# wzjin2017/fhe-fed

Hardware: AMD Instinct MI355X
Metric: ciphertexts aggregated/sec (+ encode+enc / dec+decode ms), N clients, ring 2^15 L=4 (higher is better)
Workload: dtype u64; 1 GPU; cfg3: 16 learners/GPU x ResNet-18 (11689512 params -> 714 cts of 16384 slots), ring 2^15, L=4 towers; ring_dim=32768, towers=4, learners_total=16, cts_per_learner=714, parallelism=dp1 (one GPU, no collective), layout=arena

## Files before the change

fhe-fed_amd/csrc/kernels.hip:

```cpp
#include <hip/hip_runtime.h>

#include <algorithm>
#include <cmath>
#include <cstring>
#include <type_traits>
#include <vector>

#include "dev_common.h"
#include "shelfi_internal.h"

namespace shelfi {

static uint32_t xcd_combos(uint64_t G) {
  if (!switches().xcd_order) return 0;
  return (G % 8 == 0 && G <= 0xFFFFFFFFull) ? (uint32_t)G : 0;
}

template <int LOGR>
__global__ __launch_bounds__(256) void ntt_fwd_cols(uint64_t* __restrict__ polys, uint32_t L,
                                                    uint32_t logN, const uint64_t* __restrict__ tw,
                                                    const uint64_t* __restrict__ twp,
                                                    const TowerConst* __restrict__ tcs) {
  constexpr int R = 1 << LOGR;
  const uint32_t N = 1u << logN;
// ... 280 lines not shown
      const uint64_t e = (poly == 1 ? 0 : LN) + off + (last_g(r) << K4);
#pragma unroll
      for (int m = 0; m < ML; m += 2) {
        P[r][m / 2] = *reinterpret_cast<const ulonglong2*>(pk + e + m);
        Ps[r][m / 2] = *reinterpret_cast<const ulonglong2*>(pksh + e + m);
      }
    }
  };
  uint32_t k = blockIdx.x / ncombo;
  if (k < K) fetch(k, 0);
  __syncthreads();
  const auto lds_ld = [&](uint32_t, uint32_t pj) { return sm[pj]; };
  const auto mid_sync = [] {
    if (WL)
      wave_lds_sync();
    else
      __syncthreads();
  };
#pragma unroll 1
  for (; k < K; k += per_combo) {
#pragma unroll 1
    for (int poly = 0; poly < 3; ++poly) {
      uint64_t x[NS1][M1];
      if (VT && poly == 0) {
#pragma unroll
        for (int m = 0; m < M1; ++m) {
          const uint32_t w = (uint32_t)pf[0][m];
          x[0][m] = vts[w & 127u] + vts[81 + ((w >> 7) & 127u)] + vts[162 + ((w >> 14) & 127u)] + vts[243 + (w >> 21)];
        }
      } else {
#pragma unroll
        for (int r = 0; r < NS1; ++r)
#pragma unroll
          for (int m = 0; m < M1; ++m) x[r][m] = pf[r][m];
      }
      if (poly < 2)
        fetch(k, poly + 1);
      else if (k + per_combo < K)
        fetch(k + per_combo, 0);
      if (poly > 0) fetch_key(poly);
#pragma unroll
      for (int r = 0; r < NS1; ++r)
        fwd_set_ct<BL, BL - 1, K1, NR>(x[r], 0u, tws, q, n8q);
      if (WL) __syncthreads();
#pragma unroll
      for (int r = 0; r < NS1; ++r) {
        const uint32_t p0 = lpad(threadIdx.x + 256u * r);
#pragma unroll
        for (int m = 0; m < M1; ++m) sm[p0 + lofs<(1 << D1)>(m)] = x[r][m];
      }
      __syncthreads();
      fwd_chunk_ct<BL, BL - 1 - K1, K2, NR>(tws, q, n8q, lds_ld, [&](int, uint32_t, uint32_t pj0, auto& y) {
#pragma unroll
        for (int m = 0; m < (1 << K2); ++m) sm[pj0 + lofs<(1 << (BL - K1 - K2))>(m)] = y[m];
      });
      mid_sync();
      fwd_chunk_ct<BL, BL - 1 - K1 - K2, K3, NR>(tws, q, n8q, lds_ld, [&](int, uint32_t, uint32_t pj0, auto& y) {
#pragma unroll
        for (int m = 0; m < (1 << K3); ++m) sm[pj0 + lofs<(1 << (BL - K1 - K2 - K3))>(m)] = y[m];
      });
      mid_sync();
#pragma unroll
      for (int r = 0; r < NSL; ++r) {
        const uint32_t g = last_g(r), j0 = g << K4, pj0 = lpad(j0);
        uint64_t y[ML];
#pragma unroll
        for (int m = 0; m < ML; ++m) y[m] = sm[pj0 + m];
        fwd_set_ct<BL, K4 - 1, K4, NR>(y, g, tws, q, n8q);
        if (poly == 0) {
#pragma unroll
          for (int m = 0; m < ML; ++m) V[r][m] = y[m];
        } else {
          uint64_t* __restrict__ dst = ct + ((uint64_t)k * 2 + (poly - 1)) * LN + off + j0;
#pragma unroll
          for (int m = 0; m < ML; m += 2) {
            ulonglong2 c;
            c.x = red_any(shoup_lazy(V[r][m], P[r][m / 2].x, Ps[r][m / 2].x, q) + y[m], cst);
            c.y = red_any(shoup_lazy(V[r][m + 1], P[r][m / 2].y, Ps[r][m / 2].y, q) + y[m + 1], cst);
            *reinterpret_cast<ulonglong2*>(dst + m) = c;
          }
        }
      }
      if (!WL) __syncthreads();
    }
  }
}

template <int BL, int K1, int K2, int K3, int K4, bool SUM = false>
__global__ __launch_bounds__(256) void ntt_inv_blocks_dec_ct(uint64_t* __restrict__ dbuf, uint32_t L,
                                                             uint32_t logN,
                                                             const ulonglong2* __restrict__ twb,
                                                             const TowerConst* __restrict__ tcs,
                                                             const uint64_t* __restrict__ ct,
                                                             const uint64_t* __restrict__ sk,
                                                             const uint64_t* __restrict__ sksh,
                                                             uint32_t xg, uint32_t ctL) {
  static_assert(K1 + K2 + K3 + K4 == BL, "chunk plan must cover the block");
  __shared__ __attribute__((aligned(16))) uint64_t sm[lpad_size(BL)];
  const uint32_t sstart = logN - BL;
  const uint32_t bid = xcd_block(blockIdx.x, xg);
  const uint32_t b = bid & ((1u << sstart) - 1);
  const uint32_t poly = bid >> sstart;
  const uint32_t t = poly % L, k = poly / L;
  const TowerConst& cst = tcs[t];
  const uint64_t q = cst.q, n4q = cst.n4q, n8q = cst.n8q;
  const ulonglong2* __restrict__ tb = twb + ((uint64_t)t << logN) + ((uint64_t)b << BL);
  const uint64_t off = ((uint64_t)t << logN) + ((uint64_t)b << BL);
  const uint64_t LN = (uint64_t)L << logN;
  const uint64_t CLN = (uint64_t)ctL << logN;
  const uint64_t* __restrict__ c0 = ct + (uint64_t)k * 2 * CLN + off;
  const uint64_t* __restrict__ c1 = c0 + CLN;
  const uint64_t* __restrict__ s = sk + off;
  const uint64_t* __restrict__ ss = sksh + off;
  const auto lds_ld = [&](uint32_t, uint32_t pj) { return sm[pj]; };
  inv_chunk_ct<BL, 0, K1, false>(tb, q, n8q,
                          [&](uint32_t j, uint32_t) {
                            const uint64_t a0 = SUM ? red_any(c0[j], cst) : c0[j];
                            return csub_neg(a0 + shoup_lazy(c1[j], s[j], ss[j], q), n4q);
                          },
                          [&](int, uint32_t, uint32_t pj0, auto& x) {
#pragma unroll
                            for (int m = 0; m < (1 << K1); ++m) sm[pj0 + lofs<1>(m)] = x[m];
                          });
  __syncthreads();
  inv_chunk_ct<BL, K1, K2, true>(tb, q, n8q, lds_ld, [&](int, uint32_t, uint32_t pj0, auto& x) {
#pragma unroll
    for (int m = 0; m < (1 << K2); ++m) sm[pj0 + lofs<(1 << K1)>(m)] = x[m];
  });
  __syncthreads();
  inv_chunk_ct<BL, K1 + K2, K3, true>(tb, q, n8q, lds_ld, [&](int, uint32_t, uint32_t pj0, auto& x) {
#pragma unroll
    for (int m = 0; m < (1 << K3); ++m) sm[pj0 + lofs<(1 << (K1 + K2))>(m)] = x[m];
  });
  __syncthreads();
  uint64_t* __restrict__ dst = dbuf + (uint64_t)k * LN + off;
  inv_chunk_ct<BL, BL - K4, K4, true>(tb, q, n8q, lds_ld, [&](int, uint32_t j0, uint32_t, auto& x) {
#pragma unroll
    for (int m = 0; m < (1 << K4); ++m) dst[j0 + (m << (BL - K4))] = x[m];
  });
}

template <int BL, int K1, int K2, int K3, int K4, bool SUM = false, bool WL = false>
__global__ __launch_bounds__(256) void ntt_inv_blocks_dec_pp(uint64_t* __restrict__ dbuf, uint32_t L,
                                                             uint32_t logN,
                                                             const ulonglong2* __restrict__ twb,
                                                             const TowerConst* __restrict__ tcs,
                                                             const uint64_t* __restrict__ ct,
                                                             const uint64_t* __restrict__ sk,
                                                             const uint64_t* __restrict__ sksh, uint32_t K,
                                                             uint32_t per_combo, uint32_t ctL) {
  static_assert(K1 + K2 + K3 + K4 == BL, "chunk plan must cover the block");
  constexpr int M1 = 1 << K1, NS1 = (1 << (BL - K1)) / 256;
  static_assert(!WL || (BL == 11 && K1 == 2 && K2 == 3 && K3 == 3 && K4 == 3), "wave-local plan");
  __shared__ __attribute__((aligned(16))) ulonglong2 tws[1 << BL];
  __shared__ __attribute__((aligned(16))) uint64_t sm[lpad_size(BL)];
  const auto first_g = [&](int r) -> uint32_t {
    return WL ? ((threadIdx.x >> 6) * (64u * NS1) + 64u * r + (threadIdx.x & 63u)) : threadIdx.x + 256u * r;
  };
  const uint32_t sstart = logN - BL;
  const uint32_t ncombo = L << sstart;
  const uint32_t combo = blockIdx.x % ncombo;
  const uint32_t b = combo & ((1u << sstart) - 1), t = combo >> sstart;
  const TowerConst& cst = tcs[t];
  const uint64_t q = cst.q, n4q = cst.n4q, n8q = cst.n8q;
  const uint64_t off = ((uint64_t)t << logN) + ((uint64_t)b << BL);
  const uint64_t LN = (uint64_t)L << logN;
// ... 396 lines not shown
      smc[i0 + lenh] = cmul(csub(a0, a1), W);
    }
    __syncthreads();
  }
  for (uint32_t i = threadIdx.x; i < blk; i += 256) buf[off + i] = smc[i];
}

template <int KC, int A>
__device__ __forceinline__ void fft_dit_set(double2 (&v)[1 << KC], uint32_t l, const double2* __restrict__ tw) {
#pragma unroll
  for (int i = 0; i < KC; ++i) {
#pragma unroll
    for (int m0 = 0; m0 < (1 << KC); ++m0) {
      if (m0 & (1 << i)) continue;
      const int m1 = m0 + (1 << i);
      const double2 W = tw[(1u << (A + i)) + l + ((uint32_t)(m0 & ((1 << i) - 1)) << A)];
      const double2 u = v[m0];
      const double2 w = cmul(v[m1], W);
      v[m0] = cadd(u, w);
      v[m1] = csub(u, w);
    }
  }
}
template <int KC, int A>
__device__ __forceinline__ void fft_dif_set(double2 (&v)[1 << KC], uint32_t l, const double2* __restrict__ tw) {
#pragma unroll
  for (int i = KC - 1; i >= 0; --i) {
#pragma unroll
    for (int m0 = 0; m0 < (1 << KC); ++m0) {
      if (m0 & (1 << i)) continue;
      const int m1 = m0 + (1 << i);
      const double2 W = tw[(1u << (A + i)) + l + ((uint32_t)(m0 & ((1 << i) - 1)) << A)];
      const double2 a0 = v[m0], a1 = v[m1];
      v[m0] = cadd(a0, a1);
      v[m1] = cmul(csub(a0, a1), W);
    }
  }
}
template <int BL, int KC, int A, bool DIT, class Load, class Store>
__device__ __forceinline__ void fft_chunk(const double2* __restrict__ tw, Load ld, Store st) {
  constexpr int T = 1 << (BL - 3), NS = (1 << (BL - KC)) / T;
  static_assert(NS >= 1, "chunk plan");
#pragma unroll
  for (int r = 0; r < NS; ++r) {
    const uint32_t s = threadIdx.x + (uint32_t)T * r;
    const uint32_t l = s & ((1u << A) - 1), j0 = ((s >> A) << (A + KC)) | l;
    double2 v[1 << KC];
#pragma unroll
    for (int m = 0; m < (1 << KC); ++m) v[m] = ld(j0 + ((uint32_t)m << A));
    if (DIT)
      fft_dit_set<KC, A>(v, l, tw);
    else
      fft_dif_set<KC, A>(v, l, tw);
#pragma unroll
    for (int m = 0; m < (1 << KC); ++m) st(j0 + ((uint32_t)m << A), v[m]);
  }
}
template <bool SWZ = true>
__device__ __forceinline__ uint32_t fft_swz(uint32_t j) { return SWZ ? j ^ ((j >> 3) & 15u) : j; }

template <int BL, int K1, int K2, int K3, int K4, bool SWZ = true>
__global__ __launch_bounds__(1 << (BL - 3)) void fft_inv_blocks_ct(double2* __restrict__ buf, uint32_t logS,
                                                                  const double2* __restrict__ tw) {
  static_assert(K1 + K2 + K3 + K4 == BL, "chunk plan");
  __shared__ __attribute__((aligned(16))) double2 sm[1 << BL];
  const uint32_t S = 1u << logS, sh = logS - BL;
  const uint64_t k = blockIdx.x >> sh;
  const uint32_t b = blockIdx.x & ((1u << sh) - 1);
  double2* __restrict__ g = buf + k * S + ((uint64_t)b << BL);
  const auto lds_ld = [&](uint32_t j) { return sm[fft_swz<SWZ>(j)]; };
  const auto lds_st = [&](uint32_t j, double2 v) { sm[fft_swz<SWZ>(j)] = v; };
  fft_chunk<BL, K1, BL - K1, false>(tw, [&](uint32_t j) { return g[j]; }, lds_st);
  __syncthreads();
  fft_chunk<BL, K2, BL - K1 - K2, false>(tw, lds_ld, lds_st);
  __syncthreads();
  fft_chunk<BL, K3, BL - K1 - K2 - K3, false>(tw, lds_ld, lds_st);
  __syncthreads();
  fft_chunk<BL, K4, 0, false>(tw, lds_ld, [&](uint32_t j, double2 v) { g[j] = v; });
}

constexpr uint32_t kFftWholeLogS = 14;
constexpr uint64_t kFftWholeMinK = 128;
constexpr uint64_t kEncNoredMinK = 192;
constexpr uint64_t kDecPpMinItems = 4096;
constexpr uint32_t kFftWholeRow = 1088;
__device__ __forceinline__ uint32_t fft_wpad(uint32_t e) { return e + (e >> 5); }
__device__ __forceinline__ uint32_t fft_wt1(uint32_t l, int m) { return 4 * l + (l >> 3) + 264u * (m >> 2) + (m & 3); }
__device__ __forceinline__ uint32_t fft_wx3(uint32_t l, int m) { return l + (l >> 5) + 66u * m; }
__device__ __forceinline__ uint32_t fft_xa1(uint32_t l, int m) { return 4 * l + (l >> 2) + 272u * (m >> 2) + (m & 3); }
__device__ __forceinline__ uint32_t fft_xa2(uint32_t l, int m) { return 68 * (l >> 2) + (l & 3) + 4u * m + (m >> 2); }
__device__ __forceinline__ uint32_t fft_xb2(uint32_t l, int m) {
  return 68 * (l >> 2) + (l & 3) + 4u * m + 2u * (m >> 3);
}
__device__ __forceinline__ uint32_t fft_xb3(uint32_t l, int m) { return l + 2 * (l >> 5) + 68u * m; }

template <class PF, class QF>
__device__ __forceinline__ void fft_wave_xch(double2 (&a)[16], double* __restrict__ Ls, PF P, QF Q) {
#pragma unroll
  for (int m = 0; m < 16; ++m) Ls[P(m)] = a[m].x;
  wave_lds_sync();
#pragma unroll
  for (int m = 0; m < 16; ++m) a[m].x = Ls[Q(m)];
  wave_lds_sync();
#pragma unroll
  for (int m = 0; m < 16; ++m) Ls[P(m)] = a[m].y;
  wave_lds_sync();
#pragma unroll
  for (int m = 0; m < 16; ++m) a[m].y = Ls[Q(m)];
  wave_lds_sync();
}

template <bool TO_BLOCKS>
__device__ __forceinline__ void fft_whole_transpose(double2 (&a)[16], double* __restrict__ lds) {
  const uint32_t T = threadIdx.x, w = T >> 6, l = T & 63;
#pragma unroll
  for (int part = 0; part < 2; ++part) {
#pragma unroll
    for (int i = 0; i < 16; ++i) {
      const double v = part ? a[i].y : a[i].x;
      if (TO_BLOCKS)
        lds[i * kFftWholeRow + fft_wpad(T)] = v;
      else
        lds[w * kFftWholeRow + fft_wx3(l, i)] = v;
    }
    __syncthreads();
#pragma unroll
    for (int i = 0; i < 16; ++i) {
      const double v = TO_BLOCKS ? lds[w * kFftWholeRow + fft_wx3(l, i)] : lds[i * kFftWholeRow + fft_wpad(T)];
      if (part)
        a[i].y = v;
      else
        a[i].x = v;
    }
    __syncthreads();
  }
}

__global__ __launch_bounds__(1024) void fft_inv_whole(const double* __restrict__ x, uint64_t n,
                                                      double2* __restrict__ buf, const double2* __restrict__ tw) {
  constexpr uint32_t S = 1u << kFftWholeLogS, BLK = 1024;
  constexpr int R = 16;
  __shared__ double lds[16 * kFftWholeRow];
  const uint64_t k = blockIdx.x;
  const uint32_t T = threadIdx.x, w = T >> 6, l = T & 63;
  double2 a[R];
  const double* __restrict__ xk = x + k * S;
  const uint32_t rem = n > k * S ? (uint32_t)std::min<uint64_t>(n - k * S, S) : 0u;
#pragma unroll
  for (int r = 0; r < R; ++r) {
    const uint32_t i = T + (uint32_t)r * BLK;
    a[r] = make_double2(i < rem ? xk[i] : 0.0, 0.0);
  }
#pragma unroll
  for (int s = 0; s < 4; ++s) {
    asm volatile("" ::: "memory");
    const uint32_t lenh = (S >> s) >> 1;
    const int trr = R >> (s + 1);
#pragma unroll
    for (int r0 = 0; r0 < R; ++r0) {
      if ((r0 / trr) % 2) continue;
      const int r1 = r0 + trr;
      const double2 W = tw[lenh + T + (uint32_t)(r0 & ((R >> s) - 1)) * BLK];
      const double2 u = cadd(a[r0], a[r1]);
      const double2 d = csub(a[r0], a[r1]);
      a[r0] = u;
      a[r1] = cmul(d, W);
// ... 461 lines not shown
void launch_encrypt(const Params& p, const DeviceTables& dt, const DeviceKeys& dk, const double* x,
                    uint64_t n, uint64_t K, uint64_t* ct, void* scratch, const uint32_t key[8],
                    uint64_t g0, GenFlag flag, hipStream_t s) {
  if (!K) return;
  const uint32_t logS = __builtin_ctz(p.batch);
  double2* fbuf = reinterpret_cast<double2*>(scratch);
  uint64_t* pbuf = reinterpret_cast<uint64_t*>(fbuf + K * (uint64_t)p.batch);
  launch_encode_fft(p, dt, x, n, K, fbuf, s);
  Key8 k8;
  for (int i = 0; i < 8; ++i) k8.k[i] = key[i];
  const Switches& sw = switches();
  const uint32_t nblkLog = ntt_block_log(p.logN);
  const int nlogR = (int)(p.logN - nblkLog);
  const bool fused = (nlogR == 3 || nlogR == 4 || (nlogR == 5 && sw.enc_tab && sw.enc_x5)) && dt.enc_tab &&
                     sw.enc_fused;
  int64_t* me0 = reinterpret_cast<int64_t*>(pbuf + K * 3ull * p.L * p.N);
  int16_t* ve = reinterpret_cast<int16_t*>(me0 + K * (uint64_t)p.N);
  const bool pp = fused && nblkLog == 11 && dt.red_ok && sw.enc_pp;
  uint32_t t_split = 0;
  while (t_split < p.L && p.q[t_split] >= kNoRedQ) ++t_split;
  for (uint32_t t = t_split; t < p.L; ++t)
    if (p.q[t] >= kNoRedQ) t_split = p.L;
  if (!pp || !sw.enc_nored || K < kEncNoredMinK || nlogR == 5) t_split = p.L;
  bool vt = false;
  if (fused) {
    const uint64_t nb = (K << (p.logN - (nlogR == 5 ? 4 : nlogR))) / 256;
    const bool tab = sw.enc_tab;
#define ENC_COLS(LR, TB, ...)                                                                                   \
  hipLaunchKernelGGL((enc_cols_fused<LR, TB, ##__VA_ARGS__>), dim3((uint32_t)nb), dim3(256), 0, s, fbuf, K, p.logN, logS, p.L, \
                     p.delta, dt.cdt, dt.cdt_len, k8, g0, dt.tc, dt.psi_rev, dt.psi_rev_sh, pbuf, flag, t_split,  \
                     dt.enc_tab)
    const bool ts = nlogR == 4 && tab && p.L == 4 && (sw.enc_ts >= 0 ? sw.enc_ts == 1 : K <= kEncTsMaxK);
    vt = pp && tab && !ts && nlogR == 4 && dt.enc_vtab && sw.enc_vt && ntt_wave_local();
    if (nlogR == 5)
      ENC_COLS(4, true, 3, true, false, false, true);
    else if (vt)
      ENC_COLS(4, true, 3, true, false, true);
    else if (ts)
      hipLaunchKernelGGL((enc_cols_fused<4, true, 3, true, true>), dim3((uint32_t)(nb * 4)), dim3(256), 0, s, fbuf, K,
                         p.logN, logS, p.L, p.delta, dt.cdt, dt.cdt_len, k8, g0, dt.tc, dt.psi_rev, dt.psi_rev_sh,
                         pbuf, flag, t_split, dt.enc_tab);
    else if (nlogR == 3 && tab)
      ENC_COLS(3, true);
    else if (nlogR == 3)
      ENC_COLS(3, false);
    else if (tab)
      ENC_COLS(4, true, 3, true);
    else
      ENC_COLS(4, false);
#undef ENC_COLS
    SHELFI_HIP(hipGetLastError());
  } else {
    const uint64_t threads = K * (p.N / 16);
    hipLaunchKernelGGL(enc_prep_kernel, dim3((uint32_t)((threads + 255) / 256)), dim3(256), 0, s, fbuf,
                       K, p.logN, logS, p.delta, dt.cdt, dt.cdt_len, k8, g0, me0, ve, flag);
    SHELFI_HIP(hipGetLastError());
  }
  if (nlogR > 0 && !fused) {
    const uint64_t nb = K * ((p.N >> nlogR) / 256);
#define COLS_ENC(LR)                                                                          \
  hipLaunchKernelGGL((ntt_fwd_cols_enc<LR, 0>), dim3((uint32_t)nb), dim3(256), 0, s, me0, ve, K,  \
                     p.logN, p.L, dt.tc, dt.psi_rev, dt.psi_rev_sh, pbuf);                       \
  hipLaunchKernelGGL((ntt_fwd_cols_enc<LR, 1>), dim3((uint32_t)nb), dim3(256), 0, s, me0, ve, K,  \
                     p.logN, p.L, dt.tc, dt.psi_rev, dt.psi_rev_sh, pbuf);                       \
  hipLaunchKernelGGL((ntt_fwd_cols_enc<LR, 2>), dim3((uint32_t)nb), dim3(256), 0, s, me0, ve, K,  \
                     p.logN, p.L, dt.tc, dt.psi_rev, dt.psi_rev_sh, pbuf);
    switch (nlogR) {
      case 1: COLS_ENC(1) break;
      case 2: COLS_ENC(2) break;
      case 3: COLS_ENC(3) break;
      case 4: COLS_ENC(4) break;
      case 5: COLS_ENC(5) break;
      case 6: COLS_ENC(6) break;
      default: throw Error{SHELFI_ERR_ARG, "unsupported ring dimension"};
    }
#undef COLS_ENC
    SHELFI_HIP(hipGetLastError());
  }
  const uint64_t nbb = K * p.L << nlogR;
  if (nbb > 0x7FFFFFFFull) throw Error{SHELFI_ERR_ARG, "encrypt batch too large"};
  const uint32_t xg = xcd_combos(p.L << nlogR);
  if (pp) {
    const bool wl = ntt_wave_local();
    const auto launch_pp = [&](uint32_t ta, uint32_t nt, bool nr) {
      const uint32_t ncombo = nt << nlogR;
      const uint32_t pc = pp_per_combo(ncombo, K, 3);
#define ENC_PP(NR, WL, VT)                                                                                       \
  hipLaunchKernelGGL((ntt_fwd_blocks_enc_pp<11, 3, 3, 3, 2, NR, WL, VT>), dim3(ncombo * pc), dim3(256), 0, s, pbuf, \
                     p.L, p.logN, dt.tw_fwd_blk, dt.tc, dk.pk, dk.pk_sh, ct, (uint32_t)K, pc, ta, nt, dt.enc_vtab)
      if (nr && wl && vt) ENC_PP(true, true, true);
      else if (nr && wl) ENC_PP(true, true, false);
      else if (nr) ENC_PP(true, false, false);
      else if (wl && vt) ENC_PP(false, true, true);
      else if (wl) ENC_PP(false, true, false);
      else ENC_PP(false, false, false);
#undef ENC_PP
    };
    if (t_split > 0) launch_pp(0u, t_split, false);
    if (t_split < p.L) launch_pp(t_split, p.L - t_split, true);
  } else if (nlogR > 0 && nblkLog == 11 && dt.red_ok)
    hipLaunchKernelGGL((ntt_fwd_blocks_enc_ct<11, 3, 3, 3, 2>), dim3((uint32_t)nbb), dim3(256), 0, s,
                       pbuf, p.L, p.logN, dt.tw_fwd_blk, dt.tc, dk.pk, dk.pk_sh, ct, 0u, xg);
  else if (nlogR > 0 && nblkLog == 12 && dt.red_ok)
    hipLaunchKernelGGL((ntt_fwd_blocks_enc_ct<12, 3, 3, 3, 3>), dim3((uint32_t)nbb), dim3(256), 0, s,
                       pbuf, p.L, p.logN, dt.tw_fwd_blk, dt.tc, dk.pk, dk.pk_sh, ct, 0u, xg);
  else if (nblkLog > 11)
    hipLaunchKernelGGL(ntt_fwd_blocks_enc<8>, dim3((uint32_t)nbb), dim3(256), sizeof(uint64_t) << nblkLog, s,
                     pbuf, p.L, p.logN, (uint32_t)nlogR, dt.psi_rev, dt.psi_rev_sh, dt.tc, dk.pk,
                     dk.pk_sh, ct, nlogR > 0 ? (const int64_t*)nullptr : me0,
                     nlogR > 0 ? (const int16_t*)nullptr : ve);
  else
    hipLaunchKernelGGL(ntt_fwd_blocks_enc<4>, dim3((uint32_t)nbb), dim3(256), sizeof(uint64_t) << nblkLog, s,
                     pbuf, p.L, p.logN, (uint32_t)nlogR, dt.psi_rev, dt.psi_rev_sh, dt.tc, dk.pk,
                     dk.pk_sh, ct, nlogR > 0 ? (const int64_t*)nullptr : me0,
                     nlogR > 0 ? (const int16_t*)nullptr : ve);
  SHELFI_HIP(hipGetLastError());
}

__device__ __forceinline__ int64_t enc_fit_wrap(int64_t r) {
  constexpr int64_t kMax64 = 9223372036854775295LL;
  constexpr int64_t hf = kMax64 >> 1;
  if (r > hf) return r - kMax64;
  if (r < 0 && kMax64 + r <= hf) return r + kMax64;
  return r;
}

__global__ __launch_bounds__(256) void enc_maxabs_kernel(const double2* __restrict__ fbuf, uint32_t logS,
                                                         uint64_t* __restrict__ amax) {
  const uint32_t S = 1u << logS;
  const double2* __restrict__ f = fbuf + (uint64_t)blockIdx.x * S;
  uint64_t m = 0;
  for (uint32_t i = threadIdx.x; i < S; i += 256) {
    const double2 v = f[i];
    const uint64_t a = (uint64_t)__double_as_longlong(fabs(v.x)), b = (uint64_t)__double_as_longlong(fabs(v.y));
    m = max(m, max(a, b));
  }
  __shared__ uint64_t red[256];
  red[threadIdx.x] = m;
  __syncthreads();
  for (uint32_t w = 128; w; w >>= 1) {
    if (threadIdx.x < w) red[threadIdx.x] = max(red[threadIdx.x], red[threadIdx.x + w]);
    __syncthreads();
  }
  if (threadIdx.x == 0) amax[blockIdx.x] = red[0];
}

__global__ __launch_bounds__(256) void enc_expand_approx_kernel(
    const double2* __restrict__ fbuf, uint64_t K, uint32_t logN, uint32_t logS, uint32_t L, double delta,
    const uint64_t* __restrict__ cdt, int T, Key8 key, uint64_t g0, const TowerConst* __restrict__ tcs,
    const int32_t* __restrict__ log_approx, const uint64_t* __restrict__ pw, uint64_t* __restrict__ pbuf) {
  const uint32_t N = 1u << logN, S = 1u << logS, N16 = N >> 4, V0 = N >> 6;
  __shared__ uint32_t thi[64], tlo[64];
  load_cdt32(cdt, T, thi, tlo);
  __syncthreads();
  const uint64_t gid = (uint64_t)blockIdx.x * 256 + threadIdx.x;
  const uint64_t k = gid >> (logN - 4);
  if (k >= K) return;
  const uint32_t h = (uint32_t)(gid & (N16 - 1));
  const uint64_t nonce = (1ull << 56) | (g0 + k);
  const uint32_t half = N >> 1, gapLog = logN - 1 - logS;
  const double dS = (double)S;
  const double approx = ldexp(1.0, log_approx[k]);
  uint32_t w[16];
  chacha20_block32(key, h >> 2, nonce, w);
  uint32_t u[4] = {w[4 * (h & 3)], w[4 * (h & 3) + 1], w[4 * (h & 3) + 2], w[4 * (h & 3) + 3]};
  int32_t vv[16], e0[16], e1[16];
  int64_t mm[16];
#pragma unroll
// ... 1099 lines not shown
```

fhe-fed_amd/csrc/shelfi_internal.h:

```cpp
#pragma once

#include <hip/hip_runtime.h>

#include <cstdint>
#include <cstdlib>
#include <mutex>
#include <string>
#include <vector>

#include "../../include/shelfi.h"

namespace shelfi {

typedef unsigned __int128 u128;

void set_error(const std::string& msg);
struct Error {
  int code;
  std::string msg;
};
#define SHELFI_HIP(expr)                                                             \
  do {                                                                               \
    hipError_t _e = (expr);                                                          \
    if (_e != hipSuccess)                                                            \
      throw ::shelfi::Error{SHELFI_ERR_DEVICE, std::string(#expr) + ": " +           \
                                                 hipGetErrorString(_e)};             \
  } while (0)

constexpr int kMaxTowers = 16;
constexpr int kMaxCommRanks = 16;
constexpr int kFftBlockLog = 10;
constexpr int kFftBlockLogBig = 11;
inline uint32_t fft_block_log(uint32_t logS) {
  const uint32_t b = logS >= 15 ? (uint32_t)kFftBlockLogBig : (uint32_t)kFftBlockLog;
  return logS < b ? logS : b;
}
constexpr int kNttBlockLog = 11;
constexpr int kNttBlockLogBig = 12;
inline uint32_t ntt_block_log(uint32_t logN) {
  static const uint32_t ovr = [] {
    const char* e = std::getenv("SHELFI_NTT_BLOCK_LOG_BIG");
    const int v = e ? std::atoi(e) : 0;
    return (uint32_t)((v == 11 || v == 12) ? v : 0);
  }();
  uint32_t b = logN >= 17 ? (uint32_t)kNttBlockLogBig : (uint32_t)kNttBlockLog;
  if (ovr && logN >= 16) b = ovr;
  return logN < b ? logN : b;
}

struct Switches {
  bool xcd_order = true;
  bool ntt_wl = true;
  bool fft_ct = true;
  bool fft_whole = true;
  bool enc_fused = true;
  bool enc_pp = true;
  bool dec_pp = true;
  bool enc_nored = true;
  bool enc_tab = true;
  bool enc_vt = true;
  int enc_ts = -1;
  bool dec_all_towers = false;
  bool stage_trace = false;
  bool enc_x5 = true;
  int pack_kernel = 0;
  int pack_unroll = 0;
  int pack_waves = 0;
  int wavg_rows = 0;
  uint32_t wavg_strands = 0;
  int arena_stager = -1;
  uint64_t dev_chunk_mib = 4096;
  uint64_t wavg_chunk_mib = 0;
  uint64_t stage_slot_mib = 16;
  bool h2d_direct = false;
  bool h2d_two = true;
};
const Switches& switches();
void reload_switches();

struct Params {
  uint32_t N = 0, logN = 0, L = 0, batch = 0, gap = 0, scale_bits = 0, first_mod_bits = 0;
  uint64_t q[kMaxTowers] = {0};
  uint64_t psi[kMaxTowers] = {0};
  double delta = 0.0;
  double sigma = 3.19;
};

uint64_t powmod(uint64_t a, uint64_t e, uint64_t q);
uint64_t invmod(uint64_t a, uint64_t q);
uint64_t shoup(uint64_t w, uint64_t q);
uint64_t mod_signed(int64_t v, uint64_t q);
bool is_prime(uint64_t n);
uint32_t default_ring_dim(uint32_t L, uint32_t scale_bits, uint32_t first_mod_bits, uint32_t batch);
uint32_t hybrid_dnum(uint32_t L);
double ring_dim_qbound(uint32_t L, uint32_t scale_bits, uint32_t first_mod_bits);
void generate_chain(uint32_t N, uint32_t L, uint32_t scale_bits, uint32_t first_mod_bits,
                    uint64_t* q, uint64_t* psi);
uint64_t min_root(uint64_t m, uint64_t q);
void special_primes(uint32_t N, uint32_t L, const uint64_t* q, uint32_t* dnum, uint32_t* alpha,
                    uint32_t* kP, uint64_t* p, uint64_t* ppsi);
void fft_twiddles(uint32_t slots, double* inv_re, double* inv_im, double* fwd_re, double* fwd_im);
int gauss_cdt(double sigma, uint64_t* cdt, int max_entries);
uint64_t fnv1a(const void* data, size_t n, uint64_t h = 1469598103934665603ull);

struct TowerConst {
  uint64_t q;
  uint64_t one_shoup;
  uint64_t r30, r30_shoup;
  uint64_t r60, r60_shoup;
  uint64_t r64, r64_shoup;
  uint64_t ninv, ninv_shoup;
  uint64_t qhat_inv, qhat_inv_shoup;
  double inv_q;
  uint64_t nq, n4q, n8q;
  uint32_t red_r, red_sh, red_ok;
  uint32_t crt_sh;
  float inv_q32;
  uint32_t pad32;
  uint64_t bq62;
  uint64_t ninv_qhat, ninv_qhat_shoup;
  uint64_t ninv_qhat_w1, ninv_qhat_w1_shoup;
  uint32_t crt30[7], nq30[7];
  uint64_t crt_edge[2];
};

constexpr int kEncVTab = 4 * 81, kEncETab = 128, kEncTab = kEncVTab + kEncETab;

struct DeviceTables {
  TowerConst* tc = nullptr;
  uint64_t* psi_rev = nullptr;
  uint64_t* psi_rev_sh = nullptr;
  uint64_t* ipsi_rev = nullptr;
  uint64_t* ipsi_rev_sh = nullptr;
  ulonglong2* tw_fwd_blk = nullptr;
  ulonglong2* tw_inv_blk = nullptr;
  bool red_ok = false;
  double2* fft_inv = nullptr;
  double2* fft_fwd = nullptr;
  uint64_t* cdt = nullptr;
// ... 226 lines not shown
```

fhe-fed_amd/csrc/switches.cpp:

```cpp
#include <atomic>
#include <cstdlib>
#include <cstring>
#include <initializer_list>

#include "shelfi_internal.h"

namespace shelfi {

static std::atomic<const Switches*> g_switches{nullptr};

static bool env_flag(const char* name, char off_or_on, bool dflt) {
  const char* e = getenv(name);
  return e && *e == off_or_on ? !dflt : dflt;
}
static int env_choice(const char* name, std::initializer_list<int> allowed, int dflt) {
  const char* e = getenv(name);
  if (!e) return dflt;
  const int v = atoi(e);
  for (int a : allowed)
    if (a == v) return v;
  return dflt;
}

void reload_switches() {
  Switches s;
  s.xcd_order = env_flag("SHELFI_XCD_ORDER", '0', true);
  s.ntt_wl = env_flag("SHELFI_NTT_WL", '0', true);
  s.fft_ct = env_flag("SHELFI_FFT_CT", '0', true);
  s.fft_whole = env_flag("SHELFI_FFT_WHOLE", '0', true);
  s.enc_fused = env_flag("SHELFI_ENC_FUSED_COLS", '0', true);
  s.enc_pp = env_flag("SHELFI_ENC_PP", '0', true);
  s.dec_pp = env_flag("SHELFI_DEC_PP", '0', true);
  s.enc_nored = env_flag("SHELFI_ENC_NORED", '0', true);
  s.enc_tab = env_flag("SHELFI_ENC_TAB", '0', true);
  s.enc_vt = env_flag("SHELFI_ENC_VT", '0', true);
  s.enc_ts = env_choice("SHELFI_ENC_TS", {0, 1}, -1);
  s.dec_all_towers = env_flag("SHELFI_DEC_ALL_TOWERS", '1', false);
  s.enc_x5 = env_flag("SHELFI_ENC_X5", '0', true);
  s.stage_trace = env_choice("SHELFI_STAGE_TRACE", {0, 1}, 0) == 1;
  if (const char* e = getenv("SHELFI_PACK_KERNEL")) s.pack_kernel = !strcmp(e, "v4") ? 4 : !strcmp(e, "r3") ? 3 : 0;
  s.pack_unroll = env_choice("SHELFI_PACK_UNROLL", {1, 2, 4, 8}, 0);
  s.pack_waves = env_choice("SHELFI_PACK_WAVES", {2, 8}, 0);
  s.wavg_rows = env_choice("SHELFI_WAVG_ROWS", {1, 2}, 0);
  if (const char* e = getenv("SHELFI_WAVG_STRANDS"))
    if (atoi(e) > 1 && atoi(e) <= 4096) s.wavg_strands = (uint32_t)atoi(e);
  s.arena_stager = env_choice("SHELFI_ARENA_STAGER", {0, 1}, -1);
  if (const char* e = getenv("SHELFI_DEV_CHUNK_MIB"))
    if (atoll(e) > 0) s.dev_chunk_mib = (uint64_t)atoll(e);
  if (const char* e = getenv("SHELFI_WAVG_CHUNK_MIB"))
    if (atoll(e) > 0) s.wavg_chunk_mib = (uint64_t)atoll(e);
  if (const char* e = getenv("SHELFI_STAGE_SLOT_MIB"))
    if (atoll(e) > 0 && atoll(e) <= 256) s.stage_slot_mib = (uint64_t)atoll(e);
  s.h2d_direct = env_flag("SHELFI_H2D_DIRECT", '1', false);
  s.h2d_two = env_flag("SHELFI_H2D_TWO", '0', true);
  g_switches.store(new Switches(s), std::memory_order_release);
}
const Switches& switches() { return *g_switches.load(std::memory_order_acquire); }
static const bool g_switches_read = (reload_switches(), true);

}

extern "C" {

void shelfi_reload_switches(void) { shelfi::reload_switches(); }

}
```

Baseline: 3.355 million client-ciphertexts/s.

## Add two-ciphertext-per-block encrypt NTT kernel sharing staged twiddles in LDS

Adds a 512-thread variant of the persistent encrypt forward-NTT kernel in which two 256-thread halves each process a different ciphertext. Both halves share one LDS copy of the block twiddles and value table, and the first-stage twiddles now come from LDS rather than global memory. The variant is picked by default when ring logR equals 4 and the batch holds at least 32 ciphertexts, and an env switch can override it. The goal is to halve per-ciphertext twiddle staging and global twiddle traffic and to improve occupancy through a fixed waves-per-EU hint, at the cost of more LDS per block and extra block-wide syncs.

```diff
diff --git a/fhe-fed_amd/csrc/kernels.hip b/fhe-fed_amd/csrc/kernels.hip
--- a/fhe-fed_amd/csrc/kernels.hip
+++ b/fhe-fed_amd/csrc/kernels.hip
@@ -386,6 +386,162 @@
         }
       }
       if (!WL) __syncthreads();
+    }
+  }
+}
+
+template <int BL, int K1, int K2, int K3, int K4, bool NR, bool VT>
+__global__ __launch_bounds__(512) __attribute__((amdgpu_waves_per_eu(4, 4))) void ntt_fwd_blocks_enc_pp2(
+    const uint64_t* __restrict__ pbuf, uint32_t L, uint32_t logN, const ulonglong2* __restrict__ twb,
+    const TowerConst* __restrict__ tcs, const uint64_t* __restrict__ pk, const uint64_t* __restrict__ pksh,
+    uint64_t* __restrict__ ct, uint32_t K, uint32_t per_combo, uint32_t t0, uint32_t nt,
+    const uint64_t* __restrict__ vtab) {
+  static_assert(BL == 11 && K1 == 3 && K2 == 3 && K3 == 3 && K4 == 2, "wave-local plan");
+  constexpr int M1 = 1 << K1, D1 = BL - K1;
+  constexpr int ML = 1 << K4, NSL = (1 << (BL - K4)) / 256;
+  struct Lds {
+    uint64_t vts[VT ? 4 * 81 : 2];
+    ulonglong2 tws[1 << BL];
+    uint64_t sm2[2 * lpad_size(BL)];
+  };
+  static_assert(sizeof(uint64_t[VT ? 4 * 81 : 2]) % 16 == 0, "tws stays 16-byte aligned");
+  __shared__ __attribute__((aligned(16))) Lds lds;
+  uint64_t* const vts = lds.vts;
+  ulonglong2* const tws = lds.tws;
+  uint64_t* const sm2 = lds.sm2;
+  const uint32_t h = __builtin_amdgcn_readfirstlane(threadIdx.x >> 8), tid = threadIdx.x & 255u;
+  const auto otid = [&]() -> uint32_t {
+    uint32_t tl = tid;
+    asm volatile("" : "+v"(tl));
+    return tl & 255u;
+  };
+  constexpr int DL2 = BL - K1 - K2, DL3 = BL - K1 - K2 - K3;
+  const uint32_t hb = h * lpad_size(BL);
+  const uint32_t pj1 = hb + lpad(tid);
+  const uint32_t pj2 = hb + lpad(((tid >> DL2) << (DL2 + K2)) + (tid & ((1u << DL2) - 1)));
+  const uint32_t pj3 = hb + lpad(((tid >> DL3) << (DL3 + K3)) + (tid & ((1u << DL3) - 1)));
+  const uint32_t pjl = hb + lpad(((tid >> 6) * (64u * NSL) + (tid & 63u)) << K4);
+  constexpr uint32_t kLastStep = (64u << K4) + ((64u << K4) >> 3);
+  const auto last_g = [](uint32_t tl, int r) -> uint32_t { return (tl >> 6) * (64u * NSL) + 64u * r + (tl & 63u); };
+  const uint32_t sstart = logN - BL;
+  const uint32_t ncombo = nt << sstart;
+  const uint32_t combo = blockIdx.x % ncombo;
+  const uint32_t b = combo & ((1u << sstart) - 1), t = t0 + (combo >> sstart);
+  const TowerConst& cst = tcs[t];
+  const uint64_t q = cst.q, n8q = cst.n8q;
+  const uint64_t off = ((uint64_t)t << logN) + ((uint64_t)b << BL);
+  const uint64_t LN = (uint64_t)L << logN;
+  {
+    const ulonglong2* __restrict__ src = twb + off;
+    for (uint32_t i = threadIdx.x; i < (1u << BL); i += 512) tws[i] = src[i];
+    if (VT)
+      for (uint32_t i = threadIdx.x; i < 4 * 81; i += 512) vts[i] = vtab[((uint64_t)t * 16 + b) * (4 * 81) + i];
+  }
+  uint64_t pf[M1];
+  uint64_t V[NSL][ML];
+  const auto fetch = [&](uint32_t kk, int poly) {
+    const uint32_t tl = otid();
+    if (VT && poly == 0) {
+      const uint32_t* __restrict__ vp = reinterpret_cast<const uint32_t*>(pbuf + (uint64_t)kk * 3 * LN);
+#pragma unroll
+      for (int m = 0; m < M1; ++m) pf[m] = (vp + (m << D1))[tl];
+      return;
+    }
+    const uint64_t* __restrict__ src = pbuf + ((uint64_t)kk * 3 + poly) * LN + off;
+#pragma unroll
+    for (int m = 0; m < M1; ++m) pf[m] = __builtin_nontemporal_load((src + (m << D1)) + tl);
+  };
+  const uint32_t stride = 2 * per_combo;
+  uint32_t k0 = 2 * (blockIdx.x / ncombo);
+  if (k0 + h < K) fetch(k0 + h, 0);
+  __syncthreads();
+#pragma unroll 1
+  for (; k0 < K; k0 += stride) {
+    const uint32_t k = k0 + h;
+    const bool act = k < K;
+#pragma unroll 1
+    for (int poly = 0; poly < 3; ++poly) {
+      uint64_t x[M1];
+      if (act) {
+        if (VT && poly == 0) {
+#pragma unroll
+          for (int m = 0; m < M1; ++m) {
+            const uint32_t w = (uint32_t)pf[m];
+            x[m] = vts[w & 127u] + vts[81 + ((w >> 7) & 127u)] + vts[162 + ((w >> 14) & 127u)] + vts[243 + (w >> 21)];
+          }
+        } else {
+#pragma unroll
+          for (int m = 0; m < M1; ++m) x[m] = pf[m];
+        }
+        if (poly < 2)
+          fetch(k, poly + 1);
+        else if (k + stride < K)
+          fetch(k + stride, 0);
+        fwd_set_ct<BL, BL - 1, K1, NR>(x, 0u, tws, q, n8q);
+      }
+      __syncthreads();
+      if (act) {
+#pragma unroll
+        for (int m = 0; m < M1; ++m) sm2[pj1 + lofs<(1 << D1)>(m)] = x[m];
+      }
+      __syncthreads();
+      if (act) {
+        {
+          uint64_t y[1 << K2];
+#pragma unroll
+          for (int m = 0; m < (1 << K2); ++m) y[m] = sm2[pj2 + lofs<(1 << DL2)>(m)];
+          fwd_set_ct<BL, BL - 1 - K1, K2, NR>(y, tid >> DL2, tws, q, n8q);
+#pragma unroll
+          for (int m = 0; m < (1 << K2); ++m) sm2[pj2 + lofs<(1 << DL2)>(m)] = y[m];
+        }
+        wave_lds_sync();
+        {
+          uint64_t y[1 << K3];
+#pragma unroll
+          for (int m = 0; m < (1 << K3); ++m) y[m] = sm2[pj3 + lofs<(1 << DL3)>(m)];
+          fwd_set_ct<BL, BL - 1 - K1 - K2, K3, NR>(y, tid >> DL3, tws, q, n8q);
+#pragma unroll
+          for (int m = 0; m < (1 << K3); ++m) sm2[pj3 + lofs<(1 << DL3)>(m)] = y[m];
+        }
+        wave_lds_sync();
+        const uint32_t tl = otid();
+        const auto last_set = [&](int r, uint64_t (&y)[ML]) {
+#pragma unroll
+          for (int m = 0; m < ML; ++m) y[m] = sm2[pjl + r * kLastStep + m];
+          fwd_set_ct<BL, K4 - 1, K4, NR>(y, last_g(tl, r), tws, q, n8q);
+        };
+        if (poly == 0) {
+#pragma unroll
+          for (int r = 0; r < NSL; ++r) last_set(r, V[r]);
+        } else {
+          ulonglong2 P[NSL][ML / 2], Ps[NSL][ML / 2];
+          const uint64_t* __restrict__ kb = pk + (poly == 1 ? 0 : LN) + off;
+          const uint64_t* __restrict__ ks = pksh + (poly == 1 ? 0 : LN) + off;
+#pragma unroll
+          for (int r = 0; r < NSL; ++r) {
+            const uint32_t e = last_g(tl, r) << K4;
+#pragma unroll
+            for (int m = 0; m < ML; m += 2) {
+              P[r][m / 2] = *reinterpret_cast<const ulonglong2*>(kb + (e + m));
+              Ps[r][m / 2] = *reinterpret_cast<const ulonglong2*>(ks + (e + m));
+            }
+          }
+          uint64_t* __restrict__ dst = ct + ((uint64_t)k * 2 + (poly - 1)) * LN + off;
+#pragma unroll
+          for (int r = 0; r < NSL; ++r) {
+            uint64_t y[ML];
+            last_set(r, y);
+            const uint32_t j0 = last_g(tl, r) << K4;
+#pragma unroll
+            for (int m = 0; m < ML; m += 2) {
+              ulonglong2 c;
+              c.x = red_any(shoup_lazy(V[r][m], P[r][m / 2].x, Ps[r][m / 2].x, q) + y[m], cst);
+              c.y = red_any(shoup_lazy(V[r][m + 1], P[r][m / 2].y, Ps[r][m / 2].y, q) + y[m + 1], cst);
+              *reinterpret_cast<ulonglong2*>(dst + (j0 + m)) = c;
+            }
+          }
+        }
+      }
     }
   }
 }
@@ -948,6 +1104,7 @@
 constexpr uint32_t kFftWholeLogS = 14;
 constexpr uint64_t kFftWholeMinK = 128;
 constexpr uint64_t kEncNoredMinK = 192;
+constexpr uint64_t kEncPp2MinK = 32;
 constexpr uint64_t kDecPpMinItems = 4096;
 constexpr uint32_t kFftWholeRow = 1088;
 __device__ __forceinline__ uint32_t fft_wpad(uint32_t e) { return e + (e >> 5); }
@@ -1575,8 +1732,21 @@
   const uint32_t xg = xcd_combos(p.L << nlogR);
   if (pp) {
     const bool wl = ntt_wave_local();
+    const bool pp2 = wl && (sw.enc_pp2 >= 0 ? sw.enc_pp2 == 1 : nlogR == 4 && K >= kEncPp2MinK);
     const auto launch_pp = [&](uint32_t ta, uint32_t nt, bool nr) {
       const uint32_t ncombo = nt << nlogR;
+      if (pp2) {
+        const uint32_t pc = pp_per_combo(ncombo, (K + 1) / 2, 2);
+#define ENC_PP2(NR, VT)                                                                                        \
+  hipLaunchKernelGGL((ntt_fwd_blocks_enc_pp2<11, 3, 3, 3, 2, NR, VT>), dim3(ncombo * pc), dim3(512), 0, s, pbuf, \
+                     p.L, p.logN, dt.tw_fwd_blk, dt.tc, dk.pk, dk.pk_sh, ct, (uint32_t)K, pc, ta, nt, dt.enc_vtab)
+        if (nr && vt) ENC_PP2(true, true);
+        else if (nr) ENC_PP2(true, false);
+        else if (vt) ENC_PP2(false, true);
+        else ENC_PP2(false, false);
+#undef ENC_PP2
+        return;
+      }
       const uint32_t pc = pp_per_combo(ncombo, K, 3);
 #define ENC_PP(NR, WL, VT)                                                                                       \
   hipLaunchKernelGGL((ntt_fwd_blocks_enc_pp<11, 3, 3, 3, 2, NR, WL, VT>), dim3(ncombo * pc), dim3(256), 0, s, pbuf, \
diff --git a/fhe-fed_amd/csrc/shelfi_internal.h b/fhe-fed_amd/csrc/shelfi_internal.h
--- a/fhe-fed_amd/csrc/shelfi_internal.h
+++ b/fhe-fed_amd/csrc/shelfi_internal.h
@@ -55,6 +55,7 @@
   bool fft_whole = true;
   bool enc_fused = true;
   bool enc_pp = true;
+  int enc_pp2 = -1;
   bool dec_pp = true;
   bool enc_nored = true;
   bool enc_tab = true;
diff --git a/fhe-fed_amd/csrc/switches.cpp b/fhe-fed_amd/csrc/switches.cpp
--- a/fhe-fed_amd/csrc/switches.cpp
+++ b/fhe-fed_amd/csrc/switches.cpp
@@ -30,6 +30,7 @@
   s.fft_whole = env_flag("SHELFI_FFT_WHOLE", '0', true);
   s.enc_fused = env_flag("SHELFI_ENC_FUSED_COLS", '0', true);
   s.enc_pp = env_flag("SHELFI_ENC_PP", '0', true);
+  s.enc_pp2 = env_choice("SHELFI_ENC_PP2", {0, 1}, -1);
   s.dec_pp = env_flag("SHELFI_DEC_PP", '0', true);
   s.enc_nored = env_flag("SHELFI_ENC_NORED", '0', true);
   s.enc_tab = env_flag("SHELFI_ENC_TAB", '0', true);
```

New measurement: 3.373 million client-ciphertexts/s, median of 3. No clear change (+0.5%).
